# apache/incubator-predictionio

Hardware: NVIDIA H100
Metric: ALS iterations/sec (higher is better)
Workload: dtype f32

## Files before the change

incubator-predictionio_b200/csrc/als_pair_kernel.cuh:

```cuda
#pragma once
#include <cuda_fp16.h>
#include <cuda_runtime.h>
#include <stdint.h>

#include "als_kernels.cuh"
#include "als_lockstep.cuh"

namespace pio {
namespace pr {

constexpr int KP = 64;
constexpr int CH = 8;
constexpr int RSTR = KP;
constexpr int NSTAGE = 4;
constexpr int STAGE = CH * RSTR;
constexpr int NTILE = 20;
using LL = LsLayout<KP>;
constexpr int SLOT_STRIDE = LL::STRIDE;
constexpr int VSTR = 80;
constexpr int PART_FLOATS = LL::SIZE + KP;
static_assert(NSTAGE * STAGE <= SLOT_STRIDE, "the staging ring lives in the second slot");
static_assert(NSTAGE % 2 == 0, "a loop step consumes two stages");
constexpr int W_BVEC = 2 * SLOT_STRIDE;
constexpr int W_COL = W_BVEC + 2 * VSTR;
constexpr int W_MVAL = W_COL + 2 * VSTR;
constexpr int W_FLOATS = W_MVAL + NSTAGE * CH + 8;
constexpr size_t smem_bytes(int warps) { return sizeof(float) * (size_t)W_FLOATS * warps; }

__device__ __forceinline__ int split_exponent(float vmax) {
  if (!(vmax > 0.f)) return 0;
  if (isinf(vmax)) return -63;
  int x;
  frexpf(vmax, &x);
  const int e = 15 - x;
  return e < -63 ? -63 : e > 63 ? 63 : e;
}
__device__ __forceinline__ float pow2f(int e) { return __int_as_float((127 + e) << 23); }

__global__ void __launch_bounds__(256) abs_max_kernel(const float* __restrict__ x, long long n, unsigned* out) {
  float m = 0.f;
  const long long stride = (long long)gridDim.x * blockDim.x;
  const long long i0 = (long long)blockIdx.x * blockDim.x + threadIdx.x;
  long long tail = 0;
  if ((reinterpret_cast<uintptr_t>(x) & 15) == 0) {
    const long long n4 = n >> 2;
    for (long long i = i0; i < n4; i += stride) {
      const float4 v = __ldg(reinterpret_cast<const float4*>(x) + i);
      m = fmaxf(m, fmaxf(fmaxf(fabsf(v.x), fabsf(v.y)), fmaxf(fabsf(v.z), fabsf(v.w))));
    }
    tail = 4 * n4;
  }
  for (long long i = tail + i0; i < n; i += stride) m = fmaxf(m, fabsf(__ldg(x + i)));
#pragma unroll
  for (int o = 16; o > 0; o >>= 1) m = fmaxf(m, __shfl_xor_sync(0xffffffffu, m, o));
  if ((threadIdx.x & 31) == 0) atomicMax(out, __float_as_uint(m));
}

__device__ __forceinline__ uint64_t pack2(uint32_t x, uint32_t y) {
  uint64_t r;
  asm("mov.b64 %0, {%1, %2};" : "=l"(r) : "r"(x), "r"(y));
  return r;
}
__device__ __forceinline__ void mma_f16_p(float (&d)[4], const uint32_t (&a)[4], uint64_t b) {
  asm volatile(
      "{\n .reg .b32 b0, b1;\n mov.b64 {b0, b1}, %8;\n"
      "mma.sync.aligned.m16n8k16.row.col.f32.f16.f16.f32 {%0,%1,%2,%3}, {%4,%5,%6,%7}, {b0,b1}, {%0,%1,%2,%3};\n}\n"
      : "+f"(d[0]), "+f"(d[1]), "+f"(d[2]), "+f"(d[3])
      : "r"(a[0]), "r"(a[1]), "r"(a[2]), "r"(a[3]), "l"(b));
}
__device__ __forceinline__ void mma_f16_zp(float (&d)[4], const uint32_t (&a)[4], uint64_t b) {
  asm volatile(
      "{\n .reg .b32 b0, b1;\n mov.b64 {b0, b1}, %4;\n"
      "mma.sync.aligned.m16n8k16.row.col.f32.f16.f16.f32 {%0,%1,%2,%3}, {%5,%6,%7,%8}, {b0,b1}, {%9,%9,%9,%9};\n}\n"
      : "=f"(d[0]), "=f"(d[1]), "=f"(d[2]), "=f"(d[3])
      : "l"(b), "r"(a[0]), "r"(a[1]), "r"(a[2]), "r"(a[3]), "f"(0.f));
}

__device__ __forceinline__ void split2(float a, float b, uint32_t& hi, uint32_t& lo) {
  const __half2 h = __floats2half2_rn(a, b);
  const float2 hf = __half22float2(h);
  const __half2 l = __floats2half2_rn(__fsub_rn(a, hf.x), __fsub_rn(b, hf.y));
  hi = *reinterpret_cast<const uint32_t*>(&h);
  lo = *reinterpret_cast<const uint32_t*>(&l);
}

template <bool IMPLICIT>
__device__ __forceinline__ void accumulate_row(const SolveParams& p, long long beg, long long end, float s, float unscale,
                                               const float* __restrict__ yty, float* ring, float* mval, float* slot,
                                               float* bv) {
  const int lane = threadIdx.x & 31;
  const int g = lane >> 2, t = lane & 3;
  const int nchunks = 2 * (int)((end - beg + 2 * CH - 1) / (2 * CH));
  const int prow = lane >> 4, psl = lane & 15;

  int nidx;
  float nval;
  auto prefetch_meta = [&](int c) {
    const long long e = beg + (long long)c * CH + (lane & 15);
    nidx = (c < nchunks && e < end) ? __ldg(p.idx + e) : -1;
    nval = (lane < 2 * CH && c < nchunks && e < end) ? __ldg(p.val + e) : 0.f;
  };
  auto issue = [&](int c) {
    if (c < nchunks) {
#pragma unroll
      for (int h = 0; h < 2; ++h) {
        float* sbuf = ring + ((c + h) % NSTAGE) * STAGE;
#pragma unroll
        for (int j = 0; j < 4; ++j) {
          const int r = 2 * j + prow;
          const int src = __shfl_sync(0xffffffffu, nidx, CH * h + r);
          float4* d4 = reinterpret_cast<float4*>(sbuf + r * RSTR + ((psl * 4) ^ (8 * r)));
          if (src >= 0) cp_async16(d4, p.src + (size_t)src * KP + psl * 4);
          else *d4 = make_float4(0.f, 0.f, 0.f, 0.f);
        }
      }
      if (lane < 2 * CH) mval[(c % NSTAGE) * CH + lane] = nval;
    }
    cp_async_commit();
  };

  float acc[NTILE][4];
#pragma unroll
  for (int i = 0; i < NTILE; ++i)
#pragma unroll
    for (int e = 0; e < 4; ++e) acc[i][e] = 0.f;
  float pb[4][2];
#pragma unroll
  for (int i = 0; i < 4; ++i) pb[i][0] = pb[i][1] = 0.f;

  int xo[4];
#pragma unroll
  for (int q = 0; q < 4; ++q) xo[q] = g + 8 * (q ^ t);

  prefetch_meta(0);
  issue(0);
  prefetch_meta(2);

#pragma unroll 1
  for (int c = 0; c < nchunks; c += 2) {
    cp_async_wait<0>();
    __syncwarp();
    issue(c + 2);
    prefetch_meta(c + 4);
    const float* XA = ring + (c % NSTAGE) * STAGE + t * RSTR;
    const float* XB = XA + STAGE;
    const float* mv = mval + (c % NSTAGE) * CH;
    float wb[4], sc[4];
    {
      const float r[4] = {mv[t], mv[t + 4], mv[CH + t], mv[CH + t + 4]};
#pragma unroll
      for (int q = 0; q < 4; ++q) {
        wb[q] = r[q];
        sc[q] = s;
        if (IMPLICIT) {
          const float c1 = p.alpha * fabsf(r[q]);
          sc[q] = __fmul_rn(sqrtf(c1), s);
          wb[q] = r[q] > 0.f ? 1.f + c1 : 0.f;
        }
      }
    }
    uint32_t hi[4][4], lo[4][4];
#pragma unroll
    for (int i = 0; i < 4; ++i) {
#pragma unroll
      for (int e = 0; e < 2; ++e) {
        const int q = 2 * i + e;
        const int c0 = xo[q & 3] + 32 * (q >> 2), c4 = 4 * RSTR + xo[q & 3] + 32 * (1 - (q >> 2));
        const float a0 = XA[c0], a4 = XA[c4], b0 = XB[c0], b4 = XB[c4];
        pb[i][e] = fmaf(wb[0], a0, pb[i][e]);
        pb[i][e] = fmaf(wb[1], a4, pb[i][e]);
        pb[i][e] = fmaf(wb[2], b0, pb[i][e]);
        pb[i][e] = fmaf(wb[3], b4, pb[i][e]);
        split2(__fmul_rn(a0, sc[0]), __fmul_rn(a4, sc[1]), hi[i][e], lo[i][e]);
        split2(__fmul_rn(b0, sc[2]), __fmul_rn(b4, sc[3]), hi[i][e + 2], lo[i][e + 2]);
      }
    }
#pragma unroll
    for (int j = 0; j < 8; ++j) {
      const int bi = j >> 1, be = j & 1;
      const uint64_t bh = pack2(hi[bi][be], hi[bi][be + 2]), bl = pack2(lo[bi][be], lo[bi][be + 2]);
#pragma unroll
      for (int i = bi; i < 4; ++i) {
        const int tile = i * (i + 1) + j;
        float d[4];
        mma_f16_zp(d, lo[i], bh);
        mma_f16_p(d, hi[i], bl);
        mma_f16_p(d, hi[i], bh);
        acc[tile][0] += d[0];
        acc[tile][1] += d[1];
        acc[tile][2] += d[2];
        acc[tile][3] += d[3];
      }
    }
  }
  cp_async_wait<0>();
  __syncwarp();

#pragma unroll
  for (int i = 0; i < 4; ++i)
#pragma unroll
    for (int e = 0; e < 2; ++e) {
      float v = pb[i][e];
      v += __shfl_xor_sync(0xffffffffu, v, 1);
      v += __shfl_xor_sync(0xffffffffu, v, 2);
      if (t == 0) bv[16 * i + 8 * e + g] = v;
    }
  {
    const float* yl = yty ? yty + g * KP + 2 * t : nullptr;
    int tile = 0;
#pragma unroll
    for (int i = 0; i < 4; ++i) {
#pragma unroll
      for (int j = 0; j <= 2 * i + 1; ++j, ++tile) {
        const int cb = j >> 1;
        const int cc = 8 * (j & 1) + 2 * t;
        float d0 = acc[tile][0] * unscale, d1 = acc[tile][1] * unscale;
        float d2 = acc[tile][2] * unscale, d3 = acc[tile][3] * unscale;
        if (yl) {
          const float2 y0 = __ldg(reinterpret_cast<const float2*>(yl + 16 * i * KP + 8 * j));
          const float2 y1 = __ldg(reinterpret_cast<const float2*>(yl + (16 * i + 8) * KP + 8 * j));
          d0 += y0.x; d1 += y0.y;
          d2 += y1.x; d3 += y1.y;
        }
        if (cb < i) {
          *reinterpret_cast<float2*>(slot + LL::offd(i, cb, g, cc)) = make_float2(d0, d1);
          *reinterpret_cast<float2*>(slot + LL::offd(i, cb, g + 8, cc)) = make_float2(d2, d3);
        } else {
          if (cc <= g) slot[LL::diag(i, g, cc)] = d0;
          if (cc + 1 <= g) slot[LL::diag(i, g, cc + 1)] = d1;
          if (cc <= g + 8) slot[LL::diag(i, g + 8, cc)] = d2;
          if (cc + 1 <= g + 8) slot[LL::diag(i, g + 8, cc + 1)] = d3;
        }
      }
    }
  }
  __syncwarp();
}

__device__ __forceinline__ void fill_identity(float* slot, float* bv) {
  const int lane = threadIdx.x & 31;
  for (int o = lane; o < LL::SIZE; o += 32) slot[o] = 0.f;
  __syncwarp();
  for (int r = lane; r < KP; r += 32) {
    slot[LL::at(r, r)] = 1.f;
    bv[r] = 0.f;
  }
  __syncwarp();
}

template <bool IMPLICIT, int WARPS>
__global__ void __launch_bounds__(32 * WARPS, 12 / WARPS) als_solve_pair_kernel(const SolveParams p, int n_items) {
  extern __shared__ __align__(16) float smem_all[];
  const int warp = threadIdx.x >> 5;
  float* smem = smem_all + warp * W_FLOATS;
  float* slot0 = smem;
  float* slot1 = smem + SLOT_STRIDE;
  float* ring = slot1;
  float* bvec = smem + W_BVEC;
  float* colbuf = smem + W_COL;
  float* mval = smem + W_MVAL;
  const int lane = threadIdx.x & 31;
  const int grp = lane >> 4;
  const int npairs = (n_items + 1) >> 1;
  const float c1_root_max = IMPLICIT ? sqrtf(p.alpha * __uint_as_float(__ldg(p.absmax + 1))) : 1.f;
  const int e = split_exponent(__uint_as_float(__ldg(p.absmax)) * c1_root_max);
  const float s = pow2f(e), unscale = pow2f(-2 * e);

#pragma unroll 1
  for (int base = blockIdx.x * WARPS; base < npairs; base += gridDim.x * WARPS) {
    const int pair = base + warp;
    int row0 = -1, row1 = -1;
    if (pair < npairs) {
#pragma unroll 1
      for (int h = 0; h < 2; ++h) {
        const int item = 2 * pair + h;
        float* slot = h ? slot1 : slot0;
        float* bv = bvec + h * VSTR;
        if (item >= n_items) {
          fill_identity(slot, bv);
          continue;
        }
        long long beg, end;
        if (p.partial) {
          beg = p.wl_beg[item];
          end = p.wl_end[item];
        } else {
          const int r = p.row_begin + item;
          beg = p.ptr[r];
          end = p.ptr[r + 1];
          if (h) row1 = r;
          else row0 = r;
        }
        accumulate_row<IMPLICIT>(p, beg, end, s, unscale, IMPLICIT && !p.partial ? p.yty : nullptr, ring, mval, slot, bv);
        if (p.partial) {
          float* out = p.partial + (size_t)item * PART_FLOATS;
          for (int o = lane; o < LL::SIZE / 4; o += 32)
            reinterpret_cast<float4*>(out)[o] = reinterpret_cast<const float4*>(slot)[o];
          for (int o = lane; o < KP; o += 32) out[LL::SIZE + o] = bv[o];
          __syncwarp();
        }
      }
    }
    if (p.partial) continue;
    if (WARPS > 1) __syncthreads();
    if (pair < npairs) {
      const int myrow = grp ? row1 : row0;
      const int rr = myrow < 0 ? p.row_begin : myrow;
      chol_lockstep<KP>(grp ? slot1 : slot0, bvec + grp * VSTR, p.lambda * p.nreg[rr], p.k, colbuf + grp * VSTR,
                        p.dst + (size_t)(p.dst_row_offset + rr) * KP, myrow >= 0, p.fail);
      __syncwarp();
    }
  }
}

template <bool IMPLICIT>
__global__ void __launch_bounds__(32, 12) als_finish_pair_kernel(const SolveParams p, const int* __restrict__ row_part_ptr,
                                                                  int n_rows) {
  extern __shared__ __align__(16) float smem[];
  float* bvec = smem + W_BVEC;
  float* colbuf = smem + W_COL;
  const int lane = threadIdx.x & 31;
  const int grp = lane >> 4;
  const int npairs = (n_rows + 1) >> 1;
#pragma unroll 1
  for (int pair = blockIdx.x; pair < npairs; pair += gridDim.x) {
#pragma unroll 1
    for (int h = 0; h < 2; ++h) {
      const int r = 2 * pair + h;
      float* slot = smem + h * SLOT_STRIDE;
      float* bv = bvec + h * VSTR;
      if (r >= n_rows) {
        fill_identity(slot, bv);
        continue;
      }
      const int p0 = row_part_ptr[r], p1 = row_part_ptr[r + 1];
      for (int o = lane; o < PART_FLOATS / 4; o += 32) {
        float4 s = make_float4(0.f, 0.f, 0.f, 0.f);
        for (int q = p0; q < p1; ++q) {
          const float4 v = __ldg(reinterpret_cast<const float4*>(p.partial + (size_t)q * PART_FLOATS) + o);
          s.x += v.x; s.y += v.y; s.z += v.z; s.w += v.w;
        }
        if (o < LL::SIZE / 4) reinterpret_cast<float4*>(slot)[o] = s;
        else reinterpret_cast<float4*>(bv)[o - LL::SIZE / 4] = s;
      }
      __syncwarp();
      if (IMPLICIT) {
        ls_add_yty<KP>(slot, p.yty);
        __syncwarp();
      }
    }
    const int myrow = 2 * pair + grp;
    const bool valid = myrow < n_rows;
    const int rr = valid ? myrow : 0;
    chol_lockstep<KP>(smem + grp * SLOT_STRIDE, bvec + grp * VSTR, p.lambda * p.nreg[rr], p.k, colbuf + grp * VSTR,
                      p.dst + (size_t)(p.dst_row_offset + rr) * KP, valid, p.fail);
    __syncwarp();
  }
}

}
}
```

Measured before the change: 35.54.

## Precompute confidence weights at prefetch and streamline async gather addressing

```diff
diff --git a/incubator-predictionio_b200/csrc/als_pair_kernel.cuh b/incubator-predictionio_b200/csrc/als_pair_kernel.cuh
--- a/incubator-predictionio_b200/csrc/als_pair_kernel.cuh
+++ b/incubator-predictionio_b200/csrc/als_pair_kernel.cuh
@@ -24,7 +24,7 @@
 constexpr int W_BVEC = 2 * SLOT_STRIDE;
 constexpr int W_COL = W_BVEC + 2 * VSTR;
 constexpr int W_MVAL = W_COL + 2 * VSTR;
-constexpr int W_FLOATS = W_MVAL + NSTAGE * CH + 8;
+constexpr int W_FLOATS = W_MVAL + 2 * NSTAGE * CH + 8;
 constexpr size_t smem_bytes(int warps) { return sizeof(float) * (size_t)W_FLOATS * warps; }
 
 __device__ __forceinline__ int split_exponent(float vmax) {
@@ -84,39 +84,62 @@
   lo = *reinterpret_cast<const uint32_t*>(&l);
 }
 
+__device__ __forceinline__ void cp_async16_or_zero(unsigned sdst, const void* gsrc, bool zero) {
+  asm volatile(
+      "{\n .reg .pred z;\n setp.ne.b32 z, %2, 0;\n cp.async.cg.shared.global [%0], [%1], 16, z;\n}\n"
+      ::"r"(sdst), "l"(gsrc), "r"((int)zero));
+}
+
 template <bool IMPLICIT>
 __device__ __forceinline__ void accumulate_row(const SolveParams& p, long long beg, long long end, float s, float unscale,
-                                               const float* __restrict__ yty, float* ring, float* mval, float* slot,
+                                               const float* __restrict__ yty, float* ring, float2* mval, float* slot,
                                                float* bv) {
   const int lane = threadIdx.x & 31;
   const int g = lane >> 2, t = lane & 3;
-  const int nchunks = 2 * (int)((end - beg + 2 * CH - 1) / (2 * CH));
+  const int nsteps = (int)((end - beg + 2 * CH - 1) / (2 * CH));
   const int prow = lane >> 4, psl = lane & 15;
+  const float alpha = p.alpha;
+  const float* __restrict__ src;
+  asm("add.s64 %0, %1, %2;" : "=l"(src) : "l"(p.src), "l"(16ll * psl));
+  const int* __restrict__ idx = p.idx + beg + (lane & 15);
+  const float* __restrict__ val = p.val + beg + (lane & 15);
+  int mrem = (int)(end - beg) - (lane & 15);
 
   int nidx;
-  float nval;
-  auto prefetch_meta = [&](int c) {
-    const long long e = beg + (long long)c * CH + (lane & 15);
-    nidx = (c < nchunks && e < end) ? __ldg(p.idx + e) : -1;
-    nval = (lane < 2 * CH && c < nchunks && e < end) ? __ldg(p.val + e) : 0.f;
+  float2 nconf;
+  auto prefetch_meta = [&]() {
+    const bool in = mrem > 0;
+    nidx = in ? __ldg(idx) : 0;
+    const float r = in ? __ldg(val) : 0.f;
+    idx += 2 * CH;
+    val += 2 * CH;
+    mrem -= 2 * CH;
+    if (IMPLICIT) {
+      const float c1 = __fmul_rn(alpha, fabsf(r));
+      nconf = make_float2(__fmul_rn(sqrtf(c1), s), r > 0.f ? __fadd_rn(1.f, c1) : 0.f);
+    } else {
+      nconf = make_float2(s, r);
+    }
   };
-  auto issue = [&](int c) {
-    if (c < nchunks) {
-#pragma unroll
-      for (int h = 0; h < 2; ++h) {
-        float* sbuf = ring + ((c + h) % NSTAGE) * STAGE;
-#pragma unroll
-        for (int j = 0; j < 4; ++j) {
-          const int r = 2 * j + prow;
-          const int src = __shfl_sync(0xffffffffu, nidx, CH * h + r);
-          float4* d4 = reinterpret_cast<float4*>(sbuf + r * RSTR + ((psl * 4) ^ (8 * r)));
-          if (src >= 0) cp_async16(d4, p.src + (size_t)src * KP + psl * 4);
-          else *d4 = make_float4(0.f, 0.f, 0.f, 0.f);
-        }
-      }
-      if (lane < 2 * CH) mval[(c % NSTAGE) * CH + lane] = nval;
-    }
-    cp_async_commit();
+  const unsigned ring_s = (unsigned)__cvta_generic_to_shared(ring);
+  unsigned dst[4];
+#pragma unroll
+  for (int j = 0; j < 4; ++j) {
+    const int r = 2 * j + prow;
+    dst[j] = ring_s + 4u * (unsigned)(r * RSTR + ((psl * 4) ^ (8 * r)));
+  }
+  auto issue = [&](int stage, int rem) {
+    rem -= prow;
+#pragma unroll
+    for (int h = 0; h < 2; ++h) {
+#pragma unroll
+      for (int j = 0; j < 4; ++j) {
+        const int si = __shfl_sync(0xffffffffu, nidx, CH * h + 2 * j + prow);
+        cp_async16_or_zero(dst[j] + 4u * (unsigned)((stage + h) * STAGE), src + (size_t)(unsigned)si * KP,
+                           CH * h + 2 * j >= rem);
+      }
+    }
+    if (lane < 2 * CH) mval[stage * CH + lane] = nconf;
   };
 
   float acc[NTILE][4];
@@ -128,36 +151,32 @@
 #pragma unroll
   for (int i = 0; i < 4; ++i) pb[i][0] = pb[i][1] = 0.f;
 
-  int xo[4];
-#pragma unroll
-  for (int q = 0; q < 4; ++q) xo[q] = g + 8 * (q ^ t);
-
-  prefetch_meta(0);
-  issue(0);
-  prefetch_meta(2);
-
-#pragma unroll 1
-  for (int c = 0; c < nchunks; c += 2) {
+  const float* xr[4];
+#pragma unroll
+  for (int q = 0; q < 4; ++q) xr[q] = ring + t * RSTR + g + 8 * (q ^ t);
+
+  const int len = (int)(end - beg);
+  prefetch_meta();
+  if (nsteps > 0) issue(0, len);
+  cp_async_commit();
+  prefetch_meta();
+
+#pragma unroll 1
+  for (int st = 0; st < nsteps; ++st) {
+    const int stage = 2 * (st & 1);
     cp_async_wait<0>();
     __syncwarp();
-    issue(c + 2);
-    prefetch_meta(c + 4);
-    const float* XA = ring + (c % NSTAGE) * STAGE + t * RSTR;
-    const float* XB = XA + STAGE;
-    const float* mv = mval + (c % NSTAGE) * CH;
+    if (st + 1 < nsteps) issue(2 - stage, len - 2 * CH * (st + 1));
+    cp_async_commit();
+    prefetch_meta();
     float wb[4], sc[4];
     {
-      const float r[4] = {mv[t], mv[t + 4], mv[CH + t], mv[CH + t + 4]};
-#pragma unroll
-      for (int q = 0; q < 4; ++q) {
-        wb[q] = r[q];
-        sc[q] = s;
-        if (IMPLICIT) {
-          const float c1 = p.alpha * fabsf(r[q]);
-          sc[q] = __fmul_rn(sqrtf(c1), s);
-          wb[q] = r[q] > 0.f ? 1.f + c1 : 0.f;
-        }
-      }
+      const float2* mv = mval + stage * CH;
+      const float2 m0 = mv[t], m1 = mv[t + 4], m2 = mv[CH + t], m3 = mv[CH + t + 4];
+      sc[0] = m0.x; wb[0] = m0.y;
+      sc[1] = m1.x; wb[1] = m1.y;
+      sc[2] = m2.x; wb[2] = m2.y;
+      sc[3] = m3.x; wb[3] = m3.y;
     }
     uint32_t hi[4][4], lo[4][4];
 #pragma unroll
@@ -165,8 +184,9 @@
 #pragma unroll
       for (int e = 0; e < 2; ++e) {
         const int q = 2 * i + e;
-        const int c0 = xo[q & 3] + 32 * (q >> 2), c4 = 4 * RSTR + xo[q & 3] + 32 * (1 - (q >> 2));
-        const float a0 = XA[c0], a4 = XA[c4], b0 = XB[c0], b4 = XB[c4];
+        const float* XA = xr[q & 3] + stage * STAGE;
+        const int c0 = 32 * (q >> 2), c4 = 4 * RSTR + 32 * (1 - (q >> 2));
+        const float a0 = XA[c0], a4 = XA[c4], b0 = XA[STAGE + c0], b4 = XA[STAGE + c4];
         pb[i][e] = fmaf(wb[0], a0, pb[i][e]);
         pb[i][e] = fmaf(wb[1], a4, pb[i][e]);
         pb[i][e] = fmaf(wb[2], b0, pb[i][e]);
@@ -258,7 +278,7 @@
   float* ring = slot1;
   float* bvec = smem + W_BVEC;
   float* colbuf = smem + W_COL;
-  float* mval = smem + W_MVAL;
+  float2* mval = reinterpret_cast<float2*>(smem + W_MVAL);
   const int lane = threadIdx.x & 31;
   const int grp = lane >> 4;
   const int npairs = (n_items + 1) >> 1;
```

New measurement: 36.25 (median of 6 runs). 1.02x the previous value.
